# CaptainEven/DenseBox

Measured on AMD Instinct MI355X. Metric: training patches/sec (240x240), higher is better.
Workload: dtype f16; 1 GPU; full training step (fwd + fused dense loss w/ hard-negative mining + bwd + grad all-reduce + SGD) of DenseBoxLMLOC on 240x240 patches; net=DenseBoxLMLOC, batch_per_gpu=64, global_batch=64, patch=240x240, parallelism=dp1, half_neg=11, grad_finite=True

## Files before the change

densebox_amd/_lib.py:

```python
import ctypes as C
import os

_HERE = os.path.dirname(os.path.abspath(__file__))
LIB_PATH = os.environ.get('DBX_LIB') or os.path.join(_HERE, 'csrc', 'libdensebox_hip.so')

F16, BF16, F32 = 0, 1, 2
DTYPE_ID = {'f16': F16, 'bf16': BF16, 'f32': F32}
ESIZE = {F16: 2, BF16: 2, F32: 4}

EPI_BIAS, EPI_RELU, EPI_GATE, EPI_DROPMASK, EPI_ACCUM, EPI_F32_NCHW, EPI_DROPHASH = 1, 2, 4, 8, 16, 32, 64
CONV_WFRAG = 128
K_IGEMM, K_DMA, K_BAND, K_C64, K_C8, K_WS, K_P8 = 1, 2, 3, 4, 5, 6, 7


class View(C.Structure):
    _fields_ = [('ptr', C.c_void_p), ('n', C.c_int32), ('h', C.c_int32), ('w', C.c_int32),
                ('pad', C.c_int32), ('ld', C.c_int32), ('c_off', C.c_int32), ('c', C.c_int32)]


class ConvDesc(C.Structure):
    _fields_ = [('dtype', C.c_int32), ('kh', C.c_int32), ('kw', C.c_int32), ('cpad', C.c_int32),
                ('cin_pad', C.c_int32), ('cout_pad', C.c_int32), ('epilogue', C.c_int32), ('drop_seed', C.c_uint32)]


# ... 1 lines not shown
    _fields_ = [('kernel', C.c_int32), ('tile_m', C.c_int32), ('tile_n', C.c_int32), ('w_frag', C.c_int32),
                ('name', C.c_char * 64)]


class Head2UpHalf(C.Structure):
    _fields_ = [(k, C.c_int32) for k in ('px_lo', 'px_n', 'own_lo', 'own_hi', 'ix_lo', 'ix_n')]


class Head2UpLaunch(C.Structure):
    _fields_ = [(k, C.c_int32) for k in ('head0', 'heads', 'kj', 'groups', 'blocks')]


class Head2UpPlan(C.Structure):
    _fields_ = [('fused', C.c_int32), ('halves', C.c_int32), ('half', Head2UpHalf * 2), ('launches', C.c_int32),
                ('launch', Head2UpLaunch * 4)]


class LossDesc(C.Structure):
    _fields_ = [('kind', C.c_int32), ('n', C.c_int32), ('half_neg', C.c_int32),
                ('lambda_loc', C.c_float), ('lambda_det', C.c_float), ('lambda_lm', C.c_float),
                ('use_labels', C.c_int32)]


class LossIO(C.Structure):
    _fields_ = [(k, C.c_void_p) for k in (
        'bbox', 'vertices', 'labels', 'rand_neg', 'lm_rand_neg',
        'score', 'loc', 'lm', 'rf', 'lmloc',
        'd_score', 'd_loc', 'd_lm', 'd_rf', 'd_lmloc',
        'loss', 'mask_cls', 'mask_lm', 'neg_idx', 'lm_neg_idx', 'pos_count')]

# ... 149 lines not shown
    'dbx_patch_cut': (C.c_int, [_VP, _VP, _I32, _I32, _VP, _VP]),
    'dbx_patch_plan_host': (C.c_int, [_I32, _I32, _I32, _VP, _I32, _D, _D, _D, _I32, C.POINTER(PatchGeom)]),
    'dbx_patch_draw': (C.c_int, [_I64, _I64, _I32, _I32, _VP]),
    'dbx_patch_check_tables': (C.c_int, [_VP, _I32, _VP, _I32, _VP, _I32]),
    'dbx_patch_aug_plan': (C.c_int, [C.POINTER(PatchAugIO), C.POINTER(PatchAugCfg), _I32, _VP]),
    'dbx_patch_augment': (C.c_int, [_VP, _VP, _VP, _VP, _I32, _I32, _I32, _VP, _VP]),
    'dbx_patch_aug_params_host': (C.c_int, [C.POINTER(PatchAugCfg), _I64, _I64, _VP, _VP, _I32, _VP, _VP, _VP, _VP, _VP]),
    'dbx_patch_augment_host': (C.c_int, [_VP, _VP, _VP, _I32, _I32, _VP]),
    'dbx_conv_wgrad_scratch_bytes': (_I64, [_I32, _PV, _PV, _I32, _I32]),
    'dbx_conv_wgrad': (C.c_int, [_I32, _PV, _PV, _I32, _I32, _I32, _I32, _I32, _VP, _VP, _VP, _I32, _VP]),
    'dbx_conv_wgrad_slice': (C.c_int, [_I32, _PV, _PV, _I32, _I32, _I32, _I32, _I32, _VP, _I32, _I32, _VP, _VP, _I32, _VP]),
    'dbx_conv_wgrad_pool_dz_ok': (C.c_int, [_I32, _PV, _PV, _I32, _I32]),
    'dbx_conv_wgrad_pool_dz': (C.c_int, [_I32, _PV, _VP, _I32, _PV, _PV, _I32, _I32, _I32, _I32, _I32, _VP, _VP, _VP, _I32, _I32, _VP]),
    'dbx_head2_backward_up_fused': (C.c_int, [_I32, _PV, _PV]),
    'dbx_head2_backward_up_plan': (C.c_int, [_I32, _PV, _PV, C.POINTER(C.c_int32), _I32, C.POINTER(Head2UpPlan)]),
    'dbx_heads1_wgrad_gen_ok': (C.c_int, [_I32, _PV, _I32]),
    'dbx_heads1_dgrad_gen': (C.c_int, [_I32, _PV, C.POINTER(C.c_void_p), C.POINTER(C.c_int32), _I32, _I32, C.c_uint32, _VP, _PV, _PV, _VP]),
    'dbx_heads1_wgrad_gen': (C.c_int, [_I32, _PV, _PV, C.POINTER(C.c_void_p), C.POINTER(C.c_int32), _I32, _I32, C.c_uint32, _I32, _VP, _I32, _I32,
                             _VP, _VP, _VP]),
    'dbx_conv_wgrad_plan': (C.c_int, [_I32, _PV, _PV, _I32, _I32, C.c_char_p, _I32, C.POINTER(C.c_int32)]),
    'dbx_nchw_to_framed': (C.c_int, [_I32, _VP, _I32, _PV, _VP]),
    'dbx_u8hwc_to_framed': (C.c_int, [_I32, _VP, _PV, C.POINTER(C.c_float), C.POINTER(C.c_float), _VP]),
    'dbx_nchw_to_framed_ch': (C.c_int, [_I32, _VP, _I32, _PV, _I32, _VP]),
    'dbx_nchw_to_framed_slots': (C.c_int, [_I32, _VP, _VP, _I32, _I32, _PV, _VP]),
    'dbx_framed_to_nchw_f32': (C.c_int, [_I32, _PV, _VP, _VP]),
    'dbx_framed_add_ch': (C.c_int, [_I32, _PV, _I32, _I32, _PV, _I32, _VP]),
    'dbx_maxpool2x2': (C.c_int, [_I32, _PV, _PV, _VP]),
    'dbx_maxpool2x2_bwd': (C.c_int, [_I32, _PV, _PV, _PV, _I32, _I32, _VP]),
    'dbx_maxpool_idx_bytes': (C.c_int64, [_I32, _I32, _I32, _I32]),
    'dbx_maxpool2x2_idx': (C.c_int, [_I32, _PV, _PV, _VP, _VP]),
# ... 74 lines not shown
```

densebox_amd/csrc/aux_ops.hip:

```cpp
#include "common.hpp"
#include <mutex>

static thread_local char g_err[512] = "";
void dbx_set_error(const char* fmt, ...) {
    va_list ap;
    va_start(ap, fmt);
    vsnprintf(g_err, sizeof(g_err), fmt, ap);
    va_end(ap);
}
extern "C" const char* dbx_last_error(void) { return g_err; }
extern "C" int dbx_version(void) { return DBX_ABI_VERSION; }
extern "C" int dbx_device_arch(int device) {
    hipDeviceProp_t p;
    if (hipGetDeviceProperties(&p, device) != hipSuccess) { dbx_set_error("hipGetDeviceProperties failed"); return DBX_ERR_HIP; }
    int arch = 0;
    const char* s = p.gcnArchName;
    if (s[0] == 'g' && s[1] == 'f' && s[2] == 'x') arch = (int)strtol(s + 3, nullptr, 16) == 0x950 ? 950 : (int)strtol(s + 3, nullptr, 10);
    return arch;
}

template <typename T> struct Vec { static constexpr int N = 16 / sizeof(T); };

template <typename T> __device__ __forceinline__ void load_vec(const T* p, float (&v)[16 / sizeof(T)]) {
    const u32x4 raw = *(const u32x4*)p;
// ... 1038 lines not shown
                                  uint32_t drop_seed, float* const* dw, float* const* db, void* scratch, void* stream) {
    if (!d_out || !hid || !w2 || !k || !d_hid || !dw || !scratch) { dbx_set_error("head2_backward: null argument"); return DBX_ERR_ARG; }
    DBX_DISPATCH_DTYPE(dtype, head2_wgrad_t, d_out, hid, k, nh, dw, db, scratch, (hipStream_t)stream, w2, d_hid, dropmask, dropmask_ld,
                       use_hash, (unsigned)drop_seed);
}

#ifndef H2U_D
#define H2U_D 2
#endif
#ifndef H2U_NB
#define H2U_NB 4
#endif
#ifndef H2U_WGS
#define H2U_WGS 512
#endif
struct H2UHalf { int px_lo, px_n, own_lo, own_hi, ix_lo, ix_n; };
struct H2UPlan { int halves; H2UHalf h[2]; };
template <typename T, int KJ>
__global__ __launch_bounds__(256, 2) void head2_backward_up_kernel(FrameGeo dout, FrameGeo hid, FrameGeo dhid, FrameGeo dg, int hd0, int nhl, int slot,
                                                                   Head2Args ha, float* __restrict__ partial, float* __restrict__ bpartial,
                                                                   const unsigned char* __restrict__ mask, int mask_ld, int use_hash,
                                                                   unsigned drop_seed, float sy, float sx, H2UPlan plan, int nostore) {
    constexpr int V = 8, CS = 64, LPP = CS / V, D = H2U_D, PW = 32, NB = H2U_NB, NT = 6;
    static_assert(sizeof(T) == 2, "16-bit element types");
    __shared__ int s_x0[64], s_lo[32], s_hi[32];
    __shared__ float s_l0[64], s_l1[64];
    extern __shared__ __attribute__((aligned(16))) char h2u_smem[];
    float* const s_v = (float*)h2u_smem;
    const int nsl = nhl * (512 / CS), H = hid.h, W = hid.w;
    int b = blockIdx.x;
    const int sl = b % nsl; b /= nsl;
    const int half = b % plan.halves, grp = b / plan.halves, G = gridDim.x / (nsl * plan.halves);
    const H2UHalf hf = half ? plan.h[1] : plan.h[0];
    const int hd = hd0 + sl / (512 / CS), cbase = (sl % (512 / CS)) * CS;
    const int pl = threadIdx.x / LPP, ch = threadIdx.x % LPP, c0 = cbase + ch * V;
    const int px = hf.px_lo + pl;
    const bool active = pl < hf.px_n, owner = active && px >= hf.own_lo && px < hf.own_hi;
    if (threadIdx.x < W) {
        int x0, x1; float lx0, lx1;
        bilin_coef((int)threadIdx.x, sx, dg.w, x0, x1, lx0, lx1);
        s_x0[threadIdx.x] = x0; s_l0[threadIdx.x] = x1 == x0 ? lx0 + lx1 : lx0; s_l1[threadIdx.x] = x1 == x0 ? 0.f : lx1;
    }
    __syncthreads();
    if (threadIdx.x < hf.ix_n) {
        const int ix = hf.ix_lo + threadIdx.x;
        int lo = W, hi = -1;
        for (int ox = 0; ox < W; ++ox) { const int x0 = s_x0[ox]; if (x0 == ix || x0 == ix - 1) { if (ox < lo) lo = ox; hi = ox; } }
        s_lo[threadIdx.x] = lo; s_hi[threadIdx.x] = hi;
    }
    __syncthreads();
    const int tl = threadIdx.x / (CS / 4), tq = threadIdx.x % (CS / 4), tix = hf.ix_lo + tl;
    const bool xtask = tl < hf.ix_n;
// ... 302 lines not shown
        H2ULaunch launches[4];
        const int nl = h2u_launches(k, nh, hid->n, plan.halves, launches);
        float* const pbase = (float*)scratch;
        long long pused = 0;
        int blocks_max = 0;
        for (int li = 0; li < nl; ++li) {
            const int h0 = launches[li].h0, nhl = launches[li].nhl, h1 = h0 + nhl, nsl = nhl * 8, kj = launches[li].kj, blocks = launches[li].blocks;
            float* partial = pbase + pused;
            float* bpartial = partial + (size_t)blocks * nhl * 8 * 512;
            for (int i = h0; i < h1; ++i) { o.poff[i] = pused; o.boff[i] = pused + (long long)blocks * nhl * 8 * 512; o.nblk[i] = blocks; o.nhl[i] = nhl; o.hl[i] = i - h0; }
            pused += (long long)blocks * (nhl * 8 * 512 + 32);
            blocks_max = blocks > blocks_max ? blocks : blocks_max;
#define H2U_LAUNCH(KJ)                                                                                                              \
            hipLaunchKernelGGL((head2_backward_up_kernel<T, KJ>), dim3(blocks * nsl), dim3(256), smem, s, make_geo<T>(dout), make_geo<T>(hid),    \
                               make_geo<T>(nostore ? hid : dhid), make_geo<T>(dg), h0, nhl, dout->c / nh, ha, partial, bpartial, mask, mask_ld,    \
                               use_hash, drop_seed, sy, sx, plan, nostore ? 1 : 0)
            if (kj == 1) H2U_LAUNCH(1); else if (kj == 2) H2U_LAUNCH(2); else if (kj == 4) H2U_LAUNCH(4); else H2U_LAUNCH(8);
#undef H2U_LAUNCH
            DBX_LAUNCH_CHECK();
        }
        for (int i = nh; i < 4; ++i) { o.poff[i] = 0; o.boff[i] = 0; o.nblk[i] = 0; o.nhl[i] = 1; o.hl[i] = 0; }
        float* partial = pbase; float* bpartial = pbase;
        const int blocks = blocks_max;
        const int total = nh * 8 * 512 + nh * 8;
        hipLaunchKernelGGL(head2_wgrad_reduce_kernel, dim3((total + 63) / 64), dim3(1024), 0, s, partial, bpartial, blocks, nh, o);
        DBX_LAUNCH_CHECK();
    }
    return DBX_OK;
}
template <typename T> static int head2_up_fused_t(const dbx_view* hid, const dbx_view* dg) {
    float sy, sx;
// ... 23 lines not shown
    }
    H2ULaunch l[4];
    out->launches = h2u_launches(k, nh, hid->n, plan.halves, l);
    for (int i = 0; i < out->launches; ++i) {
        out->launch[i].head0 = l[i].h0; out->launch[i].heads = l[i].nhl; out->launch[i].kj = l[i].kj; out->launch[i].groups = l[i].groups;
        out->launch[i].blocks = l[i].blocks;
    }
    return DBX_OK;
}
extern "C" int dbx_head2_backward_up(int32_t dtype, const dbx_view* d_out, const dbx_view* hid, const float* const* w2, const int32_t* k,
                                     int32_t nh, const dbx_view* d_hid, const uint8_t* dropmask, int32_t dropmask_ld, int32_t use_hash,
                                     uint32_t drop_seed, float* const* dw, float* const* db, void* scratch, const dbx_view* d_g44, void* stream) {
    if (!d_out || !hid || !w2 || !k || !d_hid || !dw || !scratch || !d_g44) { dbx_set_error("head2_backward_up: null argument"); return DBX_ERR_ARG; }
    DBX_DISPATCH_DTYPE(dtype, head2_backward_up_t, d_out, hid, w2, k, nh, d_hid, dropmask, dropmask_ld, use_hash, (unsigned)drop_seed, dw, db,
                       scratch, d_g44, (hipStream_t)stream);
}

struct PackJob { const float* src; void* dst; int co, ci, taps, mode; long long ktot; int cin_pad, row_off, k_off, rows_lim; };
template <typename T>
__global__ void pack_multi_kernel(const PackJob* __restrict__ jobs) {
    const PackJob j = jobs[blockIdx.y];
    const int total = j.co * j.ci * j.taps, taps = j.taps, ci = j.ci;
    T* wp = (T*)j.dst;
    const bool fwd = j.mode == 0 || j.mode == 4;
    const int rl = j.mode >= 4 ? (int)j.ktot : j.rows_lim;
    if (sizeof(T) == 2 && j.mode != 2 && (fwd ? ci : j.co) % 8 == 0 && (j.k_off & 7) == 0 && (j.cin_pad & 7) == 0 && taps <= 25) {
        __shared__ float tile[8][32 * 25];
        const int ot = (j.co + 7) / 8, ctn = (ci + 31) / 32, ntiles = ot * ctn, row_f = 32 * taps;
        for (int tl = blockIdx.x; tl < ntiles; tl += gridDim.x) {
            const int o0 = (tl / ctn) * 8, c0 = (tl % ctn) * 32;
// ... 378 lines not shown
```

densebox_amd/engine.py:

```python
import ctypes as C
import os
import weakref

import torch

from . import _lib
from ._lib import View, ConvDesc, check, ptr, stream_ptr

_BACKBONE = [('conv1_1_1', 3, 64), ('conv1_2_1', 64, 64), ('conv2_1_1', 64, 128), ('conv2_2_1', 128, 128),
             ('conv3_1_1', 128, 256), ('conv3_2_1', 256, 256), ('conv3_4_1', 256, 256),
             ('conv4_1_1', 256, 512), ('conv4_2_1', 512, 512), ('conv4_3_1', 512, 512), ('conv4_4_1', 512, 512)]

_HEADS = {
    'DenseBox': [('det', 1), ('loc', 4)],
    'DenseBoxLM': [('det', 1), ('loc', 4), ('landmark', 4)],
    'DenseBoxLMLOC': [('det', 1), ('loc', 4), ('landmark', 4), ('lmloc', 8)],
}


_FWD_IO = {'conv1_1_1': ('x0', 'a11'), 'conv1_2_1': ('a11', 'a12'), 'conv2_1_1': ('p1', 'a21'), 'conv2_2_1': ('a21', 'a22'),
           'conv3_1_1': ('p2', 'a31'), 'conv3_2_1': ('a31', 'a32'), 'conv3_4_1': ('a32', 'c34'), 'conv4_1_1': ('p3', 'a41'),
           'conv4_2_1': ('a41', 'a42'), 'conv4_3_1': ('a42', 'a43'), 'conv4_4_1': ('a43', 'a44')}
_BWD_IO = {'conv4_4_1': ('d_a44', 'd_a43'), 'conv4_3_1': ('d_a43', 'd_a42'), 'conv4_2_1': ('d_a42', 'd_a41'),
           'conv4_1_1': ('d_a41', 'd_p3'), 'conv3_4_1': ('d_c34', 'd_a32'), 'conv3_2_1': ('d_a32', 'd_a31'),
# ... 153 lines not shown
        self.kind = net.KIND
        self.L = _lib.lib()
        self.plans = {}
        self.wcache = {}
        self.bias_cache = {}
        self.last_plan = None
        self.grad_sink = None
        self.profile = None
        self._defer = None
        self._defer_keep = []
        self._table_keys = set()
        self._tables = {}
        self._wsig = None
        self._plans_conv = {}
        self.act_hook = None

    def grad_order(self):
        heads = _HEADS[self.kind]
        names = []
        if self.kind != 'DenseBox':
            for s_ in ('conv6_3_det', 'conv6_2_det', 'conv6_1_det'):
                names += [s_ + '.weight', s_ + '.bias']
        for s_, _ in heads:
            names += ['conv5_2_%s.weight' % s_, 'conv5_2_%s.bias' % s_]
        names += ['conv5_1_%s.weight' % s_ for s_, _ in heads] + ['conv5_1_%s.bias' % s_ for s_, _ in heads]
        for s_, _, _ in reversed(_BACKBONE):
            names += [s_ + '.weight', s_ + '.bias']
        return names

    def _param(self, name):
# ... 861 lines not shown
        if gen and dt != _lib.F32:
            dhid_v = View(None, hv.n, hv.h, hv.w, 1, 512 * nh, 0, 512 * nh)
        else:
            dhid_v = self._d_hid(P).view()
        w2p = (C.c_void_p * nh)(*[w.data_ptr() for w in w2s])
        if side is not None:
            def run_h2():
                check(L.dbx_head2_wgrad(dt, C.byref(B['d_out'].view()), C.byref(hv), ks, nh,
                                        (C.c_void_p * nh)(*[t.data_ptr() for t in dw2]), (C.c_void_p * nh)(*[t.data_ptr() for t in db2]),
                                        ptr(self._h2_scratch), stream_ptr()))
                if sink is not None:
                    sink.ready(h2_names)
            on_side(run_h2)
            check(L.dbx_head2_dgrad(dt, C.byref(B['d_out'].view()), (C.c_void_p * nh)(*[w.data_ptr() for w in w2s]), ks, nh,
                                    C.byref(dhid_v), mask_p, 512 * nh, hash_on, hash_seed, s))
        elif lin:
            check(L.dbx_head2_backward_up(dt, C.byref(B['d_out'].view()), C.byref(hv), (C.c_void_p * nh)(*[w.data_ptr() for w in w2s]), ks, nh,
                                          C.byref(dhid_v), mask_p, 512 * nh, hash_on, hash_seed,
                                          (C.c_void_p * nh)(*[t.data_ptr() for t in dw2]), (C.c_void_p * nh)(*[t.data_ptr() for t in db2]),
                                          ptr(self._h2_scratch), C.byref(B['d_g44'].view()), s))
            up_done = True
            if gen and dt == _lib.F32:
                bh = P.B['d_hid']
                P.ws[bh.off:bh.off + bh.bytes].view(torch.float32).fill_(float('nan'))
        else:
            check(L.dbx_head2_backward(dt, C.byref(B['d_out'].view()), C.byref(hv), (C.c_void_p * nh)(*[w.data_ptr() for w in w2s]), ks, nh,
                                       C.byref(dhid_v), mask_p, 512 * nh, hash_on, hash_seed,
                                       (C.c_void_p * nh)(*[t.data_ptr() for t in dw2]), (C.c_void_p * nh)(*[t.data_ptr() for t in db2]),
                                       ptr(self._h2_scratch), s))
            if sink is not None:
# ... 147 lines not shown
```

include/densebox_hip.h:

```cpp
#ifndef DENSEBOX_HIP_H
#define DENSEBOX_HIP_H

#include <stdint.h>

#ifdef __cplusplus
extern "C" {
#endif

enum dbx_status {
    DBX_OK = 0,
    DBX_ERR_ARG = -1,
    DBX_ERR_HIP = -2,
    DBX_ERR_DTYPE = -3
};

enum dbx_dtype { DBX_F16 = 0, DBX_BF16 = 1, DBX_F32 = 2 };

const char* dbx_last_error(void);
#define DBX_ABI_VERSION 13
int dbx_version(void);
int dbx_device_arch(int device);

typedef struct dbx_view {
    void*   ptr;
// ... 80 lines not shown
int dbx_conv_wgrad_pool_dz_ok(int32_t dtype, const dbx_view* dz, const dbx_view* x, int32_t kh, int32_t kw);
int dbx_conv_wgrad_pool_dz(int32_t dtype, const dbx_view* dy, const void* idx, int32_t idx_channels, const dbx_view* dz, const dbx_view* x,
                           int32_t kh, int32_t kw, int32_t cpad, int32_t co, int32_t ci, float* dw_oihw, float* db, void* scratch,
                           int32_t accumulate, int32_t write_dz, void* stream);
int dbx_head2_backward_up_fused(int32_t dtype, const dbx_view* hid, const dbx_view* d_g44);
typedef struct dbx_head2_up_half { int32_t px_lo, px_n, own_lo, own_hi, ix_lo, ix_n; } dbx_head2_up_half;
typedef struct dbx_head2_up_launch { int32_t head0, heads, kj, groups, blocks; } dbx_head2_up_launch;
typedef struct dbx_head2_up_plan_t {
    int32_t fused, halves;
    dbx_head2_up_half half[2];
    int32_t launches;
    dbx_head2_up_launch launch[4];
} dbx_head2_up_plan_t;
int dbx_head2_backward_up_plan(int32_t dtype, const dbx_view* hid, const dbx_view* d_g44, const int32_t* k, int32_t nh,
                               dbx_head2_up_plan_t* out);
int dbx_heads1_wgrad_gen_ok(int32_t dtype, const dbx_view* x, int32_t nh);
int dbx_heads1_wgrad_gen(int32_t dtype, const dbx_view* d_out, const dbx_view* x, const float* const* w2, const int32_t* k, int32_t nh,
                         int32_t use_hash, uint32_t drop_seed, int32_t ci, float* dw_oihw, int32_t dw_ci_total, int32_t dw_ci_off,
                         float* db, void* scratch, void* stream);
int dbx_heads1_dgrad_gen(int32_t dtype, const dbx_view* d_out, const float* const* w2, const int32_t* k, int32_t nh, int32_t use_hash,
                         uint32_t drop_seed, const void* w1t_frag, const dbx_view* y, const dbx_view* gate, void* stream);

int dbx_fold_heads(const float* w2, const float* b2, const float* w1, const float* b1, int32_t k, float* w_out,
                   float* b_out, void* stream);
int dbx_fold_refine(const float* w1, const float* b1, const float* w2, const float* b2, const float* w3, const float* b3,
                    int32_t ci, int32_t cm, float* w_out, float* b_out, float* v_out, void* stream);
int dbx_refine_eval(const float* landmark_nchw, const float* score_nchw, int32_t n, int32_t h, int32_t w, const float* w_fold,
                    const float* b_fold, float* out_small, void* stream);
int dbx_upsample_bilinear_nchw_f32(const float* x, int32_t planes, int32_t hi, int32_t wi, float* y, int32_t ho, int32_t wo,
                                   void* stream);
// ... 314 lines not shown
```

Before: 7723 patches/s.

## Add sparse-row head2 backward path that skips pixels with zero loss gradient

Adds a sparse path for the head2 backward/upsample step of the loc and lmloc heads. Flag and list kernels find pixels whose output gradient is nonzero, and a row-gather kernel computes weight grads and hidden grads only for those pixels. If the nonzero count is above a threshold (npix/32), a device-side flag makes the existing dense kernel run instead. The path is enabled by default for 16-bit dtypes. It adds extra scan and list launches and scratch memory, and only pays off when the regression-head gradients are sparse, which the loss masking should make true.

```diff
diff --git a/densebox_amd/_lib.py b/densebox_amd/_lib.py
--- a/densebox_amd/_lib.py
+++ b/densebox_amd/_lib.py
@@ -39,6 +39,14 @@
 class Head2UpPlan(C.Structure):
     _fields_ = [('fused', C.c_int32), ('halves', C.c_int32), ('half', Head2UpHalf * 2), ('launches', C.c_int32),
                 ('launch', Head2UpLaunch * 4)]
+
+
+class Head2RowsPlan(C.Structure):
+    _fields_ = [('rows', C.c_int32), ('threshold', C.c_int32), ('launches', C.c_int32), ('launch', Head2UpLaunch * 4), ('sparse', C.c_int32),
+                ('sparse_head', C.c_int32 * 4), ('sparse_kj', C.c_int32 * 4), ('dense_blocks', C.c_int32 * 4), ('rows_blocks', C.c_int32 * 4)]
+
+
+HEAD2_PATH_ROWS, HEAD2_PATH_DENSE = 1, 2
 
 
 class LossDesc(C.Structure):
@@ -218,6 +226,10 @@
     'dbx_conv_wgrad_pool_dz': (C.c_int, [_I32, _PV, _VP, _I32, _PV, _PV, _I32, _I32, _I32, _I32, _I32, _VP, _VP, _VP, _I32, _I32, _VP]),
     'dbx_head2_backward_up_fused': (C.c_int, [_I32, _PV, _PV]),
     'dbx_head2_backward_up_plan': (C.c_int, [_I32, _PV, _PV, C.POINTER(C.c_int32), _I32, C.POINTER(Head2UpPlan)]),
+    'dbx_head2_backward_up_rows_scratch_bytes': (_I64, [_I32, _I32, _I32, _I32]),
+    'dbx_head2_backward_up_rows': (C.c_int, [_I32, _PV, _PV, C.POINTER(C.c_void_p), C.POINTER(C.c_int32), _I32, _PV, _VP, _I32, _I32, C.c_uint32,
+                                             C.POINTER(C.c_void_p), C.POINTER(C.c_void_p), _VP, _PV, C.c_uint32, _VP, _VP]),
+    'dbx_head2_backward_up_rows_plan': (C.c_int, [_I32, _PV, _PV, C.POINTER(C.c_int32), _I32, C.c_uint32, C.POINTER(Head2RowsPlan)]),
     'dbx_heads1_wgrad_gen_ok': (C.c_int, [_I32, _PV, _I32]),
     'dbx_heads1_dgrad_gen': (C.c_int, [_I32, _PV, C.POINTER(C.c_void_p), C.POINTER(C.c_int32), _I32, _I32, C.c_uint32, _VP, _PV, _PV, _VP]),
     'dbx_heads1_wgrad_gen': (C.c_int, [_I32, _PV, _PV, C.POINTER(C.c_void_p), C.POINTER(C.c_int32), _I32, _I32, C.c_uint32, _I32, _VP, _I32, _I32,
diff --git a/densebox_amd/csrc/aux_ops.hip b/densebox_amd/csrc/aux_ops.hip
--- a/densebox_amd/csrc/aux_ops.hip
+++ b/densebox_amd/csrc/aux_ops.hip
@@ -1076,13 +1076,16 @@
 #ifndef H2U_WGS
 #define H2U_WGS 512
 #endif
+#define H2R_PATH_ROWS 1
+#define H2R_PATH_DENSE 2
 struct H2UHalf { int px_lo, px_n, own_lo, own_hi, ix_lo, ix_n; };
 struct H2UPlan { int halves; H2UHalf h[2]; };
 template <typename T, int KJ>
 __global__ __launch_bounds__(256, 2) void head2_backward_up_kernel(FrameGeo dout, FrameGeo hid, FrameGeo dhid, FrameGeo dg, int hd0, int nhl, int slot,
                                                                    Head2Args ha, float* __restrict__ partial, float* __restrict__ bpartial,
                                                                    const unsigned char* __restrict__ mask, int mask_ld, int use_hash,
-                                                                   unsigned drop_seed, float sy, float sx, H2UPlan plan, int nostore) {
+                                                                   unsigned drop_seed, float sy, float sx, H2UPlan plan, int nostore,
+                                                                   const int* __restrict__ skip) {
     constexpr int V = 8, CS = 64, LPP = CS / V, D = H2U_D, PW = 32, NB = H2U_NB, NT = 6;
     static_assert(sizeof(T) == 2, "16-bit element types");
     __shared__ int s_x0[64], s_lo[32], s_hi[32];
@@ -1098,6 +1101,7 @@
     const int pl = threadIdx.x / LPP, ch = threadIdx.x % LPP, c0 = cbase + ch * V;
     const int px = hf.px_lo + pl;
     const bool active = pl < hf.px_n, owner = active && px >= hf.own_lo && px < hf.own_hi;
+    if (skip && *skip == H2R_PATH_ROWS) return;
     if (threadIdx.x < W) {
         int x0, x1; float lx0, lx1;
         bilin_coef((int)threadIdx.x, sx, dg.w, x0, x1, lx0, lx1);
@@ -1430,7 +1434,7 @@
 #define H2U_LAUNCH(KJ)                                                                                                              \
             hipLaunchKernelGGL((head2_backward_up_kernel<T, KJ>), dim3(blocks * nsl), dim3(256), smem, s, make_geo<T>(dout), make_geo<T>(hid),    \
                                make_geo<T>(nostore ? hid : dhid), make_geo<T>(dg), h0, nhl, dout->c / nh, ha, partial, bpartial, mask, mask_ld,    \
-                               use_hash, drop_seed, sy, sx, plan, nostore ? 1 : 0)
+                               use_hash, drop_seed, sy, sx, plan, nostore ? 1 : 0, (const int*)nullptr)
             if (kj == 1) H2U_LAUNCH(1); else if (kj == 2) H2U_LAUNCH(2); else if (kj == 4) H2U_LAUNCH(4); else H2U_LAUNCH(8);
 #undef H2U_LAUNCH
             DBX_LAUNCH_CHECK();
@@ -1484,6 +1488,543 @@
     if (!d_out || !hid || !w2 || !k || !d_hid || !dw || !scratch || !d_g44) { dbx_set_error("head2_backward_up: null argument"); return DBX_ERR_ARG; }
     DBX_DISPATCH_DTYPE(dtype, head2_backward_up_t, d_out, hid, w2, k, nh, d_hid, dropmask, dropmask_ld, use_hash, (unsigned)drop_seed, dw, db,
                        scratch, d_g44, (hipStream_t)stream);
+}
+
+#define H2R_SEG 256
+#define H2R_RB 256
+#define H2R_THR_MIN 16
+#define H2R_THR_DIV 32
+struct H2RScan { int nsp; int head[4]; int k[4]; };
+struct H2RRows { int hd[4], groups[4], blocks[4]; long long poff[4], boff[4]; };
+struct H2RLayout { long long hdr, segcnt, flags, map, list, dh, part, total; int npix, nseg, thr, cap, rb; };
+static inline long long h2r_align(long long x) { return (x + 255) / 256 * 256; }
+static bool h2r_layout(int n, int h, int w, int nh, H2RLayout& L) {
+    const long long npix = (long long)n * h * w;
+    if (n < 1 || h < 1 || w < 1 || nh < 1 || nh > 4 || npix > (1ll << 28)) return false;
+    L.npix = (int)npix; L.nseg = (int)((npix + H2R_SEG - 1) / H2R_SEG);
+    static int div = 0;
+    if (!div) { const char* e = getenv("DBX_HEAD2_ROWS_THR_DIV"); div = e && atoi(e) >= 1 ? atoi(e) : H2R_THR_DIV; }
+    L.thr = (int)(npix / div) > H2R_THR_MIN ? (int)(npix / div) : H2R_THR_MIN;
+    L.cap = L.thr; L.rb = L.cap < H2R_RB ? L.cap : H2R_RB;
+    long long off = 0;
+    L.hdr = off; off += 256;
+    L.segcnt = off; off += h2r_align((long long)nh * L.nseg * 4);
+    L.flags = off; off += h2r_align(npix);
+    L.map = off; off += h2r_align((long long)nh * npix * 4);
+    L.list = off; off += h2r_align((long long)nh * L.cap * 4);
+    L.dh = off; off += h2r_align((long long)nh * L.cap * 512 * 2);
+    const int dmax = 2 * n < 64 ? 2 * n : 64;
+    L.part = off; off += h2r_align((long long)nh * (dmax + L.rb) * (4096 + 32) * 4);
+    L.total = off;
+    return true;
+}
+extern "C" int64_t dbx_head2_backward_up_rows_scratch_bytes(int32_t n, int32_t h, int32_t w, int32_t nh) {
+    H2RLayout L;
+    return h2r_layout(n, h, w, nh, L) ? (int64_t)L.total : 0;
+}
+
+template <typename T>
+__global__ __launch_bounds__(256) void head2_rows_flag_kernel(FrameGeo dout, int slot, H2RScan sc, unsigned char* __restrict__ flags,
+                                                              int* __restrict__ segcnt, int nseg) {
+    static_assert(sizeof(T) == 2, "16-bit element types");
+    __shared__ int wc[4][4];
+    const int npix = dout.n * dout.h * dout.w;
+    const int p = blockIdx.x * H2R_SEG + threadIdx.x, lane = threadIdx.x & 63, wave = threadIdx.x >> 6;
+    unsigned f = 0;
+    if (p < npix) {
+        const int hw = dout.h * dout.w, n = p / hw, rem = p - n * hw, y = rem / dout.w, x = rem - y * dout.w;
+        const T* g = (const T*)dout.base + geo_pix(dout, n, y, x);
+#pragma unroll
+        for (int s = 0; s < 4; ++s) {
+            if (s < sc.nsp) {
+                const u32x4 raw = *(const u32x4*)(g + sc.head[s] * slot);
+                const unsigned short* e = (const unsigned short*)&raw;
+                bool nz = false;
+#pragma unroll
+                for (int j = 0; j < 8; ++j) nz = nz || (j < sc.k[s] && (e[j] & 0x7fffu) != 0);
+                if (nz) f |= 1u << s;
+            }
+        }
+        flags[p] = (unsigned char)f;
+    }
+#pragma unroll
+    for (int s = 0; s < 4; ++s) {
+        const unsigned long long b = __ballot((f >> s) & 1u);
+        if (lane == 0) wc[s][wave] = __popcll(b);
+    }
+    __syncthreads();
+    if ((int)threadIdx.x < sc.nsp) segcnt[(size_t)threadIdx.x * nseg + blockIdx.x] = (wc[threadIdx.x][0] + wc[threadIdx.x][1]) + (wc[threadIdx.x][2] + wc[threadIdx.x][3]);
+}
+__global__ __launch_bounds__(256) void head2_rows_list_kernel(const unsigned char* __restrict__ flags, const int* __restrict__ segcnt, int nseg, int npix,
+                                                              H2RScan sc, int thr, int cap, int* __restrict__ hdr, int* __restrict__ list,
+                                                              int* __restrict__ map) {
+    __shared__ int red[4][3][4];
+    const int p = blockIdx.x * H2R_SEG + threadIdx.x, lane = threadIdx.x & 63, wave = threadIdx.x >> 6;
+    const unsigned f = p < npix ? flags[p] : 0u;
+    int pre[4];
+#pragma unroll
+    for (int s = 0; s < 4; ++s) {
+        pre[s] = 0;
+        if (s < sc.nsp) {
+            int b = 0, t = 0;
+            for (int i = threadIdx.x; i < nseg; i += 256) { const int v = segcnt[(size_t)s * nseg + i]; t += v; if (i < (int)blockIdx.x) b += v; }
+#pragma unroll
+            for (int o = 1; o < 64; o <<= 1) { b += __shfl_xor(b, o); t += __shfl_xor(t, o); }
+            const unsigned long long bal = __ballot((f >> s) & 1u);
+            pre[s] = __popcll(bal & ((1ull << lane) - 1ull));
+            if (lane == 0) { red[s][0][wave] = b; red[s][1][wave] = t; red[s][2][wave] = __popcll(bal); }
+        }
+    }
+    __syncthreads();
+    if (blockIdx.x == 0 && threadIdx.x == 0) {
+#pragma unroll
+        for (int i = 0; i < 8; ++i) hdr[i] = 0;
+    }
+#pragma unroll
+    for (int s = 0; s < 4; ++s) {
+        if (s < sc.nsp) {
+            const int base = (red[s][0][0] + red[s][0][1]) + (red[s][0][2] + red[s][0][3]);
+            const int total = (red[s][1][0] + red[s][1][1]) + (red[s][1][2] + red[s][1][3]);
+            int woff = 0;
+#pragma unroll
+            for (int q = 0; q < 3; ++q) woff += q < wave ? red[s][2][q] : 0;
+            const int idx = base + woff + pre[s];
+            if (p < npix) {
+                const bool listed = ((f >> s) & 1u) && idx >= 0 && idx < cap;
+                map[(size_t)s * npix + p] = listed ? idx : -1;
+                if (listed) list[(size_t)s * cap + idx] = p;
+            }
+            if (blockIdx.x == 0 && threadIdx.x == 0) { hdr[2 * sc.head[s]] = total; hdr[2 * sc.head[s] + 1] = total <= thr ? H2R_PATH_ROWS : H2R_PATH_DENSE; }
+        }
+    }
+}
+template <typename T>
+__global__ __launch_bounds__(256) void head2_rows_kernel(FrameGeo dout, FrameGeo hid, int slot, Head2Args ha, H2RRows rw, const int* __restrict__ hdr,
+                                                         const int* __restrict__ map, int cap, T* __restrict__ dh, float* __restrict__ pbase,
+                                                         H2UPlan plan, int use_hash, unsigned drop_seed) {
+    static_assert(sizeof(T) == 2, "16-bit element types");
+    constexpr int V = 8, CS = 64, LPP = CS / V, TR = 64, NU = 4;
+    __shared__ int smap[NU][TR][32];
+    __shared__ unsigned long long smask[4][NU];
+    __shared__ float red[4 * 8 * CS + 32];
+    const int s = blockIdx.y;
+    int hd = rw.hd[0], G = rw.groups[0], nblk = rw.blocks[0];
+    long long poff = rw.poff[0], boff = rw.boff[0];
+#pragma unroll
+    for (int q = 1; q < 4; ++q)
+        if (s == q) { hd = rw.hd[q]; G = rw.groups[q]; nblk = rw.blocks[q]; poff = rw.poff[q]; boff = rw.boff[q]; }
+    if ((int)blockIdx.x >= nblk * (512 / CS) || hdr[2 * hd + 1] != H2R_PATH_ROWS) return;
+    float* const partial = pbase + poff;
+    float* const bpartial = pbase + boff;
+    const int count = hdr[2 * hd], nl = count < cap ? (count > 0 ? count : 0) : cap;
+    const int H = hid.h, W = hid.w, npix = hid.n * H * W;
+    int b = blockIdx.x;
+    const int sl = b % (512 / CS); b /= 512 / CS;
+    const int half = b % plan.halves, grp = b / plan.halves;
+    const H2UHalf hf = half ? plan.h[1] : plan.h[0];
+    const int cbase = sl * CS, pl = threadIdx.x / LPP, ch = threadIdx.x % LPP, c0 = cbase + ch * V;
+    const int px = hf.px_lo + pl, lane = threadIdx.x & 63, wv = threadIdx.x >> 6;
+    const bool active = pl < hf.px_n, owner = active && px >= hf.own_lo && px < hf.own_hi;
+    typedef float f32x2 __attribute__((ext_vector_type(2)));
+    float w[8][V];
+    { int k; head2_load_w<V>(ha, hd, c0, active, w, k); }
+    f32x2 w2[8][V / 2], acc[8][V / 2];
+    float bs[8];
+    const float dscale = use_hash ? 2.f : 1.f;
+#pragma unroll
+    for (int j = 0; j < 8; ++j) {
+        bs[j] = 0.f;
+#pragma unroll
+        for (int i = 0; i < V / 2; ++i) {
+            acc[j][i] = (f32x2){0.f, 0.f};
+            w2[j][i] = (f32x2){to_f32(from_f32<T>(w[j][2 * i])) * dscale, to_f32(from_f32<T>(w[j][2 * i + 1])) * dscale};
+        }
+    }
+    const int pxl = active ? px : hf.px_lo + hf.px_n - 1;
+    const int ntile = (H + TR - 1) / TR, nimg = hid.n > grp ? (hid.n - grp + G - 1) / G : 0, nunit = nimg * ntile;
+    auto unit_img = [&](int u) { return grp + (u / ntile) * G; };
+    auto unit_base = [&](int u) { return (u % ntile) * TR; };
+    for (int u0 = 0; u0 < nunit; u0 += NU) {
+        __syncthreads();
+#pragma unroll
+        for (int q = 0; q < NU; ++q) {
+            int v[8];
+            const int u = u0 + q, img = unit_img(u), base = unit_base(u);
+#pragma unroll
+            for (int t = 0; t < 8; ++t) {
+                const int e = threadIdx.x + 256 * t, r = e / 32, c = e % 32, oy = base + r, pc = hf.px_lo + c;
+                v[t] = -1;
+                if (u < nunit && oy < H && c < hf.px_n && pc < W) v[t] = map[(size_t)s * npix + ((size_t)img * H + oy) * W + pc];
+            }
+#pragma unroll
+            for (int t = 0; t < 8; ++t) {
+                const int e = threadIdx.x + 256 * t;
+                smap[q][e / 32][e % 32] = (v[t] < 0 || v[t] >= nl) ? -1 : v[t];
+            }
+        }
+        __syncthreads();
+#pragma unroll
+        for (int q = 0; q < NU; ++q) {
+            bool hit = false;
+#pragma unroll
+            for (int i = 0; i < 8; ++i) hit = hit || smap[q][lane][wv * 8 + i] >= 0;
+            const unsigned long long m = __ballot(hit);
+            if (lane == 0) smask[wv][q] = m;
+        }
+        __syncthreads();
+        int nq = 0;
+        unsigned long long nm = smask[wv][0];
+        auto next = [&](int& q, int& r) {
+            while (nm == 0ull && nq < NU - 1) { ++nq; nm = smask[wv][nq]; }
+            if (nm == 0ull) return false;
+            q = nq; r = __ffsll((long long)nm) - 1; nm &= nm - 1ull;
+            return true;
+        };
+        auto fetch = [&](int q, int r, u32x4& g, u32x4& h) {
+            const int img = unit_img(u0 + q), oy = unit_base(u0 + q) + r;
+            g = *(const u32x4*)((const T*)dout.base + geo_pix(dout, img, oy, pxl) + hd * slot);
+            h = *(const u32x4*)((const T*)hid.base + geo_pix(hid, img, oy, pxl) + hd * 512 + c0);
+        };
+        u32x4 ga = {0u, 0u, 0u, 0u}, ha_ = ga, gb = ga, hb = ga, gc = ga, hc = ga;
+        int qa = 0, ra = 0, qb = 0, rb = 0, qc = 0, rc = 0;
+        bool va = next(qa, ra);
+        if (va) fetch(qa, ra, ga, ha_);
+        bool vb = va && next(qb, rb);
+        if (vb) fetch(qb, rb, gb, hb);
+        while (va) {
+            const bool vc = vb && next(qc, rc);
+            if (vc) fetch(qc, rc, gc, hc);
+            const T* ge = (const T*)&ga;
+            const T* he = (const T*)&ha_;
+            float h[V];
+#pragma unroll
+            for (int i = 0; i < V; ++i) h[i] = to_f32(he[i]);
+            f32x2 o2[V / 2];
+#pragma unroll
+            for (int i = 0; i < V / 2; ++i) o2[i] = (f32x2){0.f, 0.f};
+#pragma unroll
+            for (int j = 0; j < 8; ++j) {
+                const float gj = to_f32(ge[j]);
+                bs[j] += gj;
+                const f32x2 g2 = {gj, gj};
+#pragma unroll
+                for (int i = 0; i < V / 2; ++i) acc[j][i] = g2 * (f32x2){h[2 * i], h[2 * i + 1]} + acc[j][i];
+#pragma unroll
+                for (int i = 0; i < V / 2; ++i) o2[i] = g2 * w2[j][i] + o2[i];
+            }
+            const int idx = smap[qa][ra][pl];
+            if (owner && idx >= 0) {
+                float o[V];
+#pragma unroll
+                for (int i = 0; i < V / 2; ++i) { o[2 * i] = o2[i].x; o[2 * i + 1] = o2[i].y; }
+                if (use_hash) {
+                    const unsigned pix = (unsigned)(((long long)unit_img(u0 + qa) * H + unit_base(u0 + qa) + ra) * W + px);
+                    const unsigned kb8 = dbx_drop_hash32(drop_seed, pix, (unsigned)(hd * 512 + c0) >> 5) >> ((unsigned)c0 & 31u);
+#pragma unroll
+                    for (int i = 0; i < V; ++i)
+                        o[i] = __builtin_bit_cast(float, __builtin_bit_cast(int, o[i]) & ((int)(kb8 << (31 - i)) >> 31));
+                }
+                u32x4 raw;
+                T* oe = (T*)&raw;
+#pragma unroll
+                for (int i = 0; i < V; ++i) oe[i] = from_f32<T>(o[i]);
+                *(u32x4*)(dh + ((size_t)s * cap + idx) * 512 + c0) = raw;
+            }
+            va = vb; qa = qb; ra = rb; ga = gb; ha_ = hb;
+            vb = vc; qb = qc; rb = rc; gb = gc; hb = hc;
+        }
+    }
+    if (!owner) {
+#pragma unroll
+        for (int j = 0; j < 8; ++j) {
+            bs[j] = 0.f;
+#pragma unroll
+            for (int i = 0; i < V / 2; ++i) acc[j][i] = (f32x2){0.f, 0.f};
+        }
+    }
+#pragma unroll
+    for (int j = 0; j < 8; ++j) {
+#pragma unroll
+        for (int i = 0; i < V; ++i) {
+            float a = acc[j][i >> 1][i & 1];
+            a += __shfl_xor(a, 8); a += __shfl_xor(a, 16); a += __shfl_xor(a, 32);
+            acc[j][i >> 1][i & 1] = a;
+        }
+        float bsum = bs[j];
+        bsum += __shfl_xor(bsum, 8); bsum += __shfl_xor(bsum, 16); bsum += __shfl_xor(bsum, 32);
+        bs[j] = bsum;
+    }
+    __syncthreads();
+    if (lane < LPP) {
+#pragma unroll
+        for (int j = 0; j < 8; ++j) {
+            *(f32x4*)&red[(wv * 8 + j) * CS + lane * V] = (f32x4){acc[j][0][0], acc[j][0][1], acc[j][1][0], acc[j][1][1]};
+            *(f32x4*)&red[(wv * 8 + j) * CS + lane * V + 4] = (f32x4){acc[j][2][0], acc[j][2][1], acc[j][3][0], acc[j][3][1]};
+        }
+        if (lane == 0) {
+#pragma unroll
+            for (int j = 0; j < 8; ++j) red[4 * 8 * CS + wv * 8 + j] = bs[j];
+        }
+    }
+    __syncthreads();
+    {
+        const size_t blk = (size_t)grp * plan.halves + half;
+        const int c = threadIdx.x % CS;
+#pragma unroll
+        for (int jj = 0; jj < 2; ++jj) {
+            const int j = threadIdx.x / CS + 4 * jj;
+            float o = 0.f;
+#pragma unroll
+            for (int q = 0; q < 4; ++q) o += red[(q * 8 + j) * CS + c];
+            partial[(blk * 8 + j) * 512 + cbase + c] = o;
+        }
+        if (cbase == 0 && threadIdx.x < 8) {
+            float bsum = 0.f;
+#pragma unroll
+            for (int q = 0; q < 4; ++q) bsum += red[4 * 8 * CS + q * 8 + threadIdx.x];
+            bpartial[blk * 32 + threadIdx.x] = bsum;
+        }
+    }
+}
+template <typename T>
+__global__ __launch_bounds__(256) void head2_rows_g44_kernel(FrameGeo hid, FrameGeo dg, H2RScan sc, const int* __restrict__ hdr, const int* __restrict__ map,
+                                                            int cap, const T* __restrict__ dh, float sy, float sx) {
+    static_assert(sizeof(T) == 2, "16-bit element types");
+    constexpr int V = 8, NT = 6;
+    const int s = blockIdx.y, lane = threadIdx.x & 63;
+    int hd = sc.head[0];
+#pragma unroll
+    for (int q = 1; q < 4; ++q)
+        if (s == q) hd = sc.head[q];
+    if (hdr[2 * hd + 1] != H2R_PATH_ROWS) return;
+    const int count = hdr[2 * hd], nl = count < cap ? count : cap;
+    const int H = hid.h, W = hid.w, hs = dg.h, ws = dg.w, npix = hid.n * H * W;
+    const long long q = (long long)blockIdx.x * 4 + (threadIdx.x >> 6);
+    if (q >= (long long)dg.n * hs * ws) return;
+    const int n = (int)(q / (hs * ws)), rem = (int)(q - (long long)n * hs * ws), iy = rem / ws, ix = rem - iy * ws;
+    int xlo = 0, nx = 0, ylo = 0, ny = 0;
+    {
+        int x0, x1; float l0, l1;
+        bilin_coef(lane, sx, ws, x0, x1, l0, l1);
+        const unsigned long long m = __ballot(lane < W && (x0 == ix || x0 == ix - 1));
+        if (m) { xlo = __ffsll((long long)m) - 1; nx = 64 - __clzll((long long)m) - xlo; nx = nx > NT ? NT : nx; }
+        bool first = true;
+        int yhi = -1;
+        for (int base = 0; base < H; base += 64) {
+            int y0, y1;
+            bilin_coef(base + lane, sy, hs, y0, y1, l0, l1);
+            const unsigned long long my = __ballot(base + lane < H && (y0 == iy || y0 == iy - 1));
+            if (my) {
+                if (first) { ylo = base + __ffsll((long long)my) - 1; first = false; }
+                yhi = base + 63 - __clzll((long long)my);
+            }
+        }
+        ny = first ? 0 : yhi - ylo + 1;
+    }
+    float c[V], Y[V];
+#pragma unroll
+    for (int i = 0; i < V; ++i) c[i] = Y[i] = 0.f;
+    int curox = -1;
+    auto close_column = [&]() {
+        int x0, x1; float l0, l1;
+        bilin_coef(curox, sx, ws, x0, x1, l0, l1);
+        const float sl0 = x1 == x0 ? l0 + l1 : l0, sl1 = x1 == x0 ? 0.f : l1;
+        const float cf = x0 == ix ? sl0 : sl1;
+#pragma unroll
+        for (int i = 0; i < V; ++i) { c[i] = fmaf(cf, Y[i], c[i]); Y[i] = 0.f; }
+    };
+    const int taps = nx * ny;
+    for (int t0 = 0; t0 < taps; t0 += 64) {
+        const int t = t0 + lane;
+        int idx = -1;
+        if (t < taps) {
+            const int ox = xlo + t / ny, oy = ylo + t % ny;
+            const long long pp = ((long long)n * H + oy) * W + ox;
+            if (ox < W && oy < H && pp < npix) idx = map[(size_t)s * npix + pp];
+        }
+        unsigned long long m = __ballot(idx >= 0 && idx < nl);
+        while (m) {
+            const int bl = __ffsll((long long)m) - 1;
+            m &= m - 1ull;
+            const int ib = __shfl(idx, bl), tb = t0 + bl, ox = xlo + tb / ny, oy = ylo + tb % ny;
+            if (ox != curox) { if (curox >= 0) close_column(); curox = ox; }
+            int y0, y1; float l0, l1;
+            bilin_coef(oy, sy, hs, y0, y1, l0, l1);
+            const float wy = (y0 == iy ? l0 : 0.f) + (y1 == iy ? l1 : 0.f);
+            const u32x4 raw = *(const u32x4*)(dh + ((size_t)s * cap + ib) * 512 + lane * V);
+            const T* e = (const T*)&raw;
+#pragma unroll
+            for (int i = 0; i < V; ++i) Y[i] = fmaf(wy, to_f32(e[i]), Y[i]);
+        }
+    }
+    if (curox >= 0) close_column();
+    u32x4 out;
+    T* oe = (T*)&out;
+#pragma unroll
+    for (int i = 0; i < V; ++i) oe[i] = from_f32<T>(c[i]);
+    *(u32x4*)((T*)dg.base + geo_pix(dg, n, iy, ix) + hd * 512 + lane * V) = out;
+}
+
+struct H2RPlan { bool rows; int nl; H2ULaunch dense[4]; H2RScan sc; H2ULaunch fb[4]; H2RLayout lay; float sy, sx; H2UPlan plan; };
+static bool h2r_plan(size_t esize, const dbx_view* hid, const dbx_view* dg, const int32_t* k, int nh, unsigned sparse, H2RPlan& R) {
+    R = H2RPlan{};
+    if (!h2u_fused(esize, hid, dg, R.sy, R.sx, R.plan) || !sparse || !h2r_layout(hid->n, hid->h, hid->w, nh, R.lay)) return false;
+    H2ULaunch full[4];
+    const int nfull = h2u_launches(k, nh, hid->n, R.plan.halves, full);
+    auto groups_of = [&](int hd) { for (int i = 0; i < nfull; ++i) if (hd >= full[i].h0 && hd < full[i].h0 + full[i].nhl) return full[i].groups; return 1; };
+    for (int h0 = 0; h0 < nh;) {
+        if (sparse >> h0 & 1u) {
+            H2ULaunch one[4];
+            h2u_launches(k + h0, 1, hid->n, R.plan.halves, one);
+            one[0].h0 = h0; one[0].groups = groups_of(h0); one[0].blocks = one[0].groups * R.plan.halves;
+            R.sc.head[R.sc.nsp] = h0; R.sc.k[R.sc.nsp] = k[h0]; R.fb[R.sc.nsp++] = one[0];
+            ++h0;
+            continue;
+        }
+        int h1 = h0 + 1;
+        while (h1 < nh && !(sparse >> h1 & 1u)) ++h1;
+        H2ULaunch run[4];
+        const int nr = h2u_launches(k + h0, h1 - h0, hid->n, R.plan.halves, run);
+        for (int i = 0; i < nr; ++i) {
+            run[i].h0 += h0; run[i].groups = groups_of(run[i].h0); run[i].blocks = run[i].groups * R.plan.halves;
+            R.dense[R.nl++] = run[i];
+        }
+        h0 = h1;
+    }
+    R.rows = true;
+    return true;
+}
+template <typename T>
+static int head2_backward_up_rows_t(const dbx_view* dout, const dbx_view* hid, const float* const* w2, const int32_t* k, int nh, const dbx_view* dhid,
+                                    const uint8_t* mask, int mask_ld, int use_hash, unsigned drop_seed, float* const* dw, float* const* db,
+                                    void* scratch, const dbx_view* dg, unsigned sparse, void* rows_scratch, hipStream_t s) {
+    DBX_REQUIRE(nh >= 1 && nh <= 4 && (sparse >> nh) == 0, "head2_backward_up_rows: nh in 1..4, sparse_heads names heads below nh only");
+    H2RPlan R;
+    const bool rows = sizeof(T) == 2 && dhid->ptr == nullptr && !mask && h2r_plan(sizeof(T), hid, dg, k, nh, sparse, R);
+    if (!rows) return head2_backward_up_t<T>(dout, hid, w2, k, nh, dhid, mask, mask_ld, use_hash, drop_seed, dw, db, scratch, dg, s);
+    if constexpr (sizeof(T) == 2) {
+        VIEW_VEC_CHECK(T, dg, "head2_backward_up_rows d_g44");
+        VIEW_VEC_CHECK(T, hid, "head2_backward_up_rows hid");
+        DBX_REQUIRE(dg->n == hid->n && dg->c == hid->c, "head2_backward_up_rows: d_g44 has the hidden map's batch and channels");
+        DBX_REQUIRE(hid->c == 512 * nh && dout->c % nh == 0 && dout->c / nh >= 8, "head2_backward_up_rows: hid of 512*nh channels, d_out of nh slots >= 8 channels");
+        DBX_REQUIRE(dout->n == hid->n && dout->h == hid->h && dout->w == hid->w && dhid->n == hid->n && dhid->h == hid->h && dhid->w == hid->w && dhid->c == hid->c,
+                    "head2_backward_up_rows: shape mismatch");
+        DBX_REQUIRE(((size_t)dout->ptr % 16) == 0 && (dout->ld * sizeof(T)) % 16 == 0 && (dout->c_off * sizeof(T)) % 16 == 0 &&
+                        ((dout->c / nh) * sizeof(T)) % 16 == 0, "head2_backward_up_rows: d_out alignment");
+        DBX_REQUIRE(((size_t)rows_scratch % 256) == 0, "head2_backward_up_rows: the rows scratch is 256-byte aligned");
+        Head2Out o;
+        Head2Args ha;
+        ha.nh = nh; ha.slot = dout->c / nh;
+        for (int i = 0; i < 4; ++i) {
+            o.dw[i] = i < nh ? dw[i] : nullptr; o.db[i] = (i < nh && db) ? db[i] : nullptr; o.k[i] = i < nh ? k[i] : 0;
+            ha.w2[i] = i < nh ? w2[i] : nullptr; ha.k[i] = i < nh ? k[i] : 0;
+            if (i < nh) DBX_REQUIRE(k[i] >= 1 && k[i] <= 8 && dw[i] && w2[i] && ((size_t)w2[i] % 16) == 0, "head2_backward_up_rows: k in 1..8, 16-byte aligned weights");
+        }
+        constexpr size_t smem = (size_t)2 * H2U_NB * 32 * 64 * 4;
+        static DbxDevOnce attr_once; int attr_dev = 0;
+        if (attr_once.pending(&attr_dev)) {
+            DBX_HIP(hipFuncSetAttribute((const void*)head2_backward_up_kernel<T, 1>, hipFuncAttributeMaxDynamicSharedMemorySize, (int)smem));
+            DBX_HIP(hipFuncSetAttribute((const void*)head2_backward_up_kernel<T, 2>, hipFuncAttributeMaxDynamicSharedMemorySize, (int)smem));
+            DBX_HIP(hipFuncSetAttribute((const void*)head2_backward_up_kernel<T, 4>, hipFuncAttributeMaxDynamicSharedMemorySize, (int)smem));
+            DBX_HIP(hipFuncSetAttribute((const void*)head2_backward_up_kernel<T, 8>, hipFuncAttributeMaxDynamicSharedMemorySize, (int)smem));
+            attr_once.mark(attr_dev);
+        }
+        const H2RLayout& Y = R.lay;
+        char* const base = (char*)rows_scratch;
+        int* const hdr = (int*)(base + Y.hdr);
+        int* const segcnt = (int*)(base + Y.segcnt);
+        unsigned char* const flags = (unsigned char*)(base + Y.flags);
+        int* const map = (int*)(base + Y.map);
+        int* const list = (int*)(base + Y.list);
+        T* const dh = (T*)(base + Y.dh);
+        float* const pbase = (float*)(base + Y.part);
+        const int slot = dout->c / nh;
+        const FrameGeo gdout = make_geo<T>(dout), ghid = make_geo<T>(hid), gdg = make_geo<T>(dg);
+        hipLaunchKernelGGL(head2_rows_flag_kernel<T>, dim3(Y.nseg), dim3(256), 0, s, gdout, slot, R.sc, flags, segcnt, Y.nseg);
+        DBX_LAUNCH_CHECK();
+        hipLaunchKernelGGL(head2_rows_list_kernel, dim3(Y.nseg), dim3(256), 0, s, flags, segcnt, Y.nseg, Y.npix, R.sc, Y.thr, Y.cap, hdr, list, map);
+        DBX_LAUNCH_CHECK();
+        long long pused = 0;
+        int blocks_max = 0;
+        auto dense_launch = [&](const H2ULaunch& L, float* partial, float* bpartial, const int* skip) {
+            const int nsl = L.nhl * 8;
+#define H2U_LAUNCH(KJ)                                                                                                              \
+            hipLaunchKernelGGL((head2_backward_up_kernel<T, KJ>), dim3(L.blocks * nsl), dim3(256), smem, s, gdout, ghid, ghid, gdg, L.h0, L.nhl, slot, \
+                               ha, partial, bpartial, (const unsigned char*)nullptr, mask_ld, use_hash, drop_seed, R.sy, R.sx, R.plan, 1, skip)
+            if (L.kj == 1) H2U_LAUNCH(1); else if (L.kj == 2) H2U_LAUNCH(2); else if (L.kj == 4) H2U_LAUNCH(4); else H2U_LAUNCH(8);
+#undef H2U_LAUNCH
+        };
+        for (int li = 0; li < R.nl; ++li) {
+            const H2ULaunch& L = R.dense[li];
+            float* partial = pbase + pused;
+            float* bpartial = partial + (size_t)L.blocks * L.nhl * 8 * 512;
+            for (int i = L.h0; i < L.h0 + L.nhl; ++i) { o.poff[i] = pused; o.boff[i] = pused + (long long)L.blocks * L.nhl * 8 * 512; o.nblk[i] = L.blocks; o.nhl[i] = L.nhl; o.hl[i] = i - L.h0; }
+            pused += (long long)L.blocks * (L.nhl * 8 * 512 + 32);
+            blocks_max = L.blocks > blocks_max ? L.blocks : blocks_max;
+            dense_launch(L, partial, bpartial, nullptr);
+            DBX_LAUNCH_CHECK();
+        }
+        for (int r = 0; r < R.sc.nsp; ++r) {
+            const int hd = R.sc.head[r], nb = R.fb[r].blocks;
+            o.poff[hd] = pused; o.boff[hd] = pused + (long long)nb * 4096; o.nblk[hd] = nb; o.nhl[hd] = 1; o.hl[hd] = 0;
+            pused += (long long)nb * (4096 + 32);
+            blocks_max = nb > blocks_max ? nb : blocks_max;
+        }
+        DBX_REQUIRE(pused * 4 <= Y.total - Y.part, "head2_backward_up_rows: partial area overflow (internal)");
+        H2RRows rw{};
+        int rows_wgs = 0;
+        for (int r = 0; r < R.sc.nsp; ++r) {
+            const int hd = R.sc.head[r];
+            rw.hd[r] = hd; rw.groups[r] = R.fb[r].groups; rw.blocks[r] = R.fb[r].blocks; rw.poff[r] = o.poff[hd]; rw.boff[r] = o.boff[hd];
+            rows_wgs = R.fb[r].blocks * 8 > rows_wgs ? R.fb[r].blocks * 8 : rows_wgs;
+        }
+        hipLaunchKernelGGL(head2_rows_kernel<T>, dim3(rows_wgs, R.sc.nsp), dim3(256), 0, s, gdout, ghid, slot, ha, rw, (const int*)hdr, (const int*)map, Y.cap, dh,
+                           pbase, R.plan, use_hash, drop_seed);
+        DBX_LAUNCH_CHECK();
+        const long long pos = (long long)dg->n * dg->h * dg->w;
+        hipLaunchKernelGGL(head2_rows_g44_kernel<T>, dim3((unsigned)((pos + 3) / 4), R.sc.nsp), dim3(256), 0, s, ghid, gdg, R.sc, (const int*)hdr, (const int*)map,
+                           Y.cap, (const T*)dh, R.sy, R.sx);
+        DBX_LAUNCH_CHECK();
+        for (int r = 0; r < R.sc.nsp; ++r) {
+            const int hd = R.sc.head[r];
+            dense_launch(R.fb[r], pbase + o.poff[hd], pbase + o.boff[hd], hdr + 2 * hd + 1);
+            DBX_LAUNCH_CHECK();
+        }
+        for (int i = nh; i < 4; ++i) { o.poff[i] = 0; o.boff[i] = 0; o.nblk[i] = 0; o.nhl[i] = 1; o.hl[i] = 0; }
+        const int total = nh * 8 * 512 + nh * 8;
+        hipLaunchKernelGGL(head2_wgrad_reduce_kernel, dim3((total + 63) / 64), dim3(1024), 0, s, pbase, pbase, blocks_max, nh, o);
+        DBX_LAUNCH_CHECK();
+    }
+    return DBX_OK;
+}
+extern "C" int dbx_head2_backward_up_rows(int32_t dtype, const dbx_view* d_out, const dbx_view* hid, const float* const* w2, const int32_t* k,
+                                          int32_t nh, const dbx_view* d_hid, const uint8_t* dropmask, int32_t dropmask_ld, int32_t use_hash,
+                                          uint32_t drop_seed, float* const* dw, float* const* db, void* scratch, const dbx_view* d_g44,
+                                          uint32_t sparse_heads, void* rows_scratch, void* stream) {
+    if (!d_out || !hid || !w2 || !k || !d_hid || !dw || !scratch || !d_g44 || !rows_scratch) { dbx_set_error("head2_backward_up_rows: null argument"); return DBX_ERR_ARG; }
+    DBX_DISPATCH_DTYPE(dtype, head2_backward_up_rows_t, d_out, hid, w2, k, nh, d_hid, dropmask, dropmask_ld, use_hash, (unsigned)drop_seed, dw, db,
+                       scratch, d_g44, (unsigned)sparse_heads, rows_scratch, (hipStream_t)stream);
+}
+extern "C" int dbx_head2_backward_up_rows_plan(int32_t dtype, const dbx_view* hid, const dbx_view* d_g44, const int32_t* k, int32_t nh,
+                                               uint32_t sparse_heads, dbx_head2_rows_plan_t* out) {
+    if (!hid || !d_g44 || !k || !out) { dbx_set_error("head2_backward_up_rows_plan: null argument"); return DBX_ERR_ARG; }
+    if (dtype != DBX_F16 && dtype != DBX_BF16 && dtype != DBX_F32) { dbx_set_error("head2_backward_up_rows_plan: unknown dtype"); return DBX_ERR_DTYPE; }
+    DBX_REQUIRE(nh >= 1 && nh <= 4 && hid->c == 512 * nh && d_g44->n == hid->n && d_g44->c == hid->c,
+                "head2_backward_up_rows_plan: nh in 1..4, hid of 512*nh channels, d_g44 with the hidden map's batch and channels");
+    DBX_REQUIRE((sparse_heads >> nh) == 0, "head2_backward_up_rows_plan: sparse_heads names heads below nh only");
+    for (int i = 0; i < nh; ++i) DBX_REQUIRE(k[i] >= 1 && k[i] <= 8, "head2_backward_up_rows_plan: k in 1..8");
+    *out = dbx_head2_rows_plan_t{};
+    H2RPlan R;
+    if (!h2r_plan(dtype == DBX_F32 ? 4 : 2, hid, d_g44, k, nh, sparse_heads, R)) return DBX_OK;
+    out->rows = 1; out->threshold = R.lay.thr; out->launches = R.nl; out->sparse = R.sc.nsp;
+    for (int i = 0; i < R.nl; ++i) {
+        out->launch[i].head0 = R.dense[i].h0; out->launch[i].heads = R.dense[i].nhl; out->launch[i].kj = R.dense[i].kj;
+        out->launch[i].groups = R.dense[i].groups; out->launch[i].blocks = R.dense[i].blocks;
+    }
+    for (int r = 0; r < R.sc.nsp; ++r) {
+        out->sparse_head[r] = R.sc.head[r]; out->sparse_kj[r] = R.fb[r].kj; out->dense_blocks[r] = R.fb[r].blocks; out->rows_blocks[r] = R.fb[r].blocks;
+    }
+    return DBX_OK;
 }
 
 struct PackJob { const float* src; void* dst; int co, ci, taps, mode; long long ktot; int cin_pad, row_off, k_off, rows_lim; };
diff --git a/densebox_amd/engine.py b/densebox_amd/engine.py
--- a/densebox_amd/engine.py
+++ b/densebox_amd/engine.py
@@ -191,6 +191,8 @@
         self._wsig = None
         self._plans_conv = {}
         self.act_hook = None
+        self.head2_rows = os.environ.get('DBX_HEAD2_ROWS', '1') != '0'
+        self._h2r_scratch = None
 
     def grad_order(self):
         heads = _HEADS[self.kind]
@@ -1082,6 +1084,16 @@
             on_side(run_h2)
             check(L.dbx_head2_dgrad(dt, C.byref(B['d_out'].view()), (C.c_void_p * nh)(*[w.data_ptr() for w in w2s]), ks, nh,
                                     C.byref(dhid_v), mask_p, 512 * nh, hash_on, hash_seed, s))
+        elif lin and gen and dt != _lib.F32 and self.head2_rows:
+            sparse = sum(1 << i for i, (st, _) in enumerate(heads) if st in ('loc', 'lmloc'))
+            need = L.dbx_head2_backward_up_rows_scratch_bytes(hv.n, hv.h, hv.w, nh)
+            if self._h2r_scratch is None or self._h2r_scratch.numel() < need or self._h2r_scratch.device != dev:
+                self._h2r_scratch = torch.empty(int(need), dtype=torch.uint8, device=dev)
+            check(L.dbx_head2_backward_up_rows(dt, C.byref(B['d_out'].view()), C.byref(hv), (C.c_void_p * nh)(*[w.data_ptr() for w in w2s]), ks, nh,
+                                               C.byref(dhid_v), mask_p, 512 * nh, hash_on, hash_seed,
+                                               (C.c_void_p * nh)(*[t.data_ptr() for t in dw2]), (C.c_void_p * nh)(*[t.data_ptr() for t in db2]),
+                                               ptr(self._h2_scratch), C.byref(B['d_g44'].view()), sparse, ptr(self._h2r_scratch), s))
+            up_done = True
         elif lin:
             check(L.dbx_head2_backward_up(dt, C.byref(B['d_out'].view()), C.byref(hv), (C.c_void_p * nh)(*[w.data_ptr() for w in w2s]), ks, nh,
                                           C.byref(dhid_v), mask_p, 512 * nh, hash_on, hash_seed,
diff --git a/include/densebox_hip.h b/include/densebox_hip.h
--- a/include/densebox_hip.h
+++ b/include/densebox_hip.h
@@ -118,6 +118,20 @@
 } dbx_head2_up_plan_t;
 int dbx_head2_backward_up_plan(int32_t dtype, const dbx_view* hid, const dbx_view* d_g44, const int32_t* k, int32_t nh,
                                dbx_head2_up_plan_t* out);
+enum { DBX_HEAD2_PATH_ROWS = 1, DBX_HEAD2_PATH_DENSE = 2 };
+typedef struct dbx_head2_rows_plan_t {
+    int32_t rows, threshold, launches;
+    dbx_head2_up_launch launch[4];
+    int32_t sparse;
+    int32_t sparse_head[4], sparse_kj[4], dense_blocks[4], rows_blocks[4];
+} dbx_head2_rows_plan_t;
+int64_t dbx_head2_backward_up_rows_scratch_bytes(int32_t n, int32_t h, int32_t w, int32_t nh);
+int dbx_head2_backward_up_rows(int32_t dtype, const dbx_view* d_out, const dbx_view* hid, const float* const* w2, const int32_t* k,
+                               int32_t nh, const dbx_view* d_hid, const uint8_t* dropmask, int32_t dropmask_ld, int32_t use_hash,
+                               uint32_t drop_seed, float* const* dw, float* const* db, void* scratch, const dbx_view* d_g44,
+                               uint32_t sparse_heads, void* rows_scratch, void* stream);
+int dbx_head2_backward_up_rows_plan(int32_t dtype, const dbx_view* hid, const dbx_view* d_g44, const int32_t* k, int32_t nh,
+                                    uint32_t sparse_heads, dbx_head2_rows_plan_t* out);
 int dbx_heads1_wgrad_gen_ok(int32_t dtype, const dbx_view* x, int32_t nh);
 int dbx_heads1_wgrad_gen(int32_t dtype, const dbx_view* d_out, const dbx_view* x, const float* const* w2, const int32_t* k, int32_t nh,
                          int32_t use_hash, uint32_t drop_seed, int32_t ci, float* dw_oihw, int32_t dw_ci_total, int32_t dw_ci_off,
```

After: 7789 patches/s, median of 6. No clear change (+0.9%).
